# microsoft/Tokenizer

Measured on AMD Instinct MI355X. Metric: input MB/s encoded (cl100k_base), higher is better.
Workload: dtype u8

## Files before the change

### tokenizer_amd/csrc/tkz_kernels.hip

```cpp
#include "tkz_kernels.h"

#include <type_traits>

#include "tkz_bpe.h"
#include "tkz_classes.h"
#include "tkz_corpus.h"
#include "tkz_pretok.h"
#include "tkz_simt.h"

namespace tkz {

TKZ_KERNEL(256) void k_docmark(const int64_t* offs, int64_t n_items, int64_t total, uint64_t* bits, int32_t* counters) {
    const int64_t stride = simt::nblocks() * simt::nthreads();
    for (int64_t d = simt::bid() * simt::nthreads() + simt::tid(); d <= n_items; d += stride) {
        const int64_t pos = offs[d];
        bool ok = pos >= 0 && pos <= total;
        if (d == 0) ok = ok && pos == 0;
        if (d == n_items) ok = ok && pos == total;
        else ok = ok && pos <= offs[d + 1];
        if (!ok) { simt::atomic_or((unsigned*)&counters[0], (unsigned)kErrOffsets); continue; }
        const int64_t w = pos >> 6;
        if (d > 0) { const int64_t prev = offs[d - 1]; if (prev >= 0 && prev <= pos && (prev >> 6) == w) continue; }
        uint64_t m = 1ull << (pos & 63);
        int64_t cur = pos;
// ... 1311 lines not shown
    int* s_cls = LD.cls;
    uint16_t* s_ord = LD.ord;
    const int lane = simt::lane();
    int err = 0;
    LongProf PF;
    tkz_long_prof_begin(P, PF);
    const int64_t nchunks = (P.nsub + 63) / 64;
    for (int64_t u = c0; u < nchunks * PARTS; u += cstep) {
        const int64_t c = u % nchunks;
        const int part = (int)(u / nchunks);
        const int64_t t = c * 64 + lane;
        int my_nl = 0;
        if (t < P.nsub) {
            const uint32_t mc = P.mcount[t];
            my_nl = (int)(mc >> 16);
            if ((int)(mc & 0xFFFFu) + my_nl > P.mcap) my_nl = 0;
            if (part == 0 && (P.heavy_flag[t] & 2u)) { const int g = P.giant_cnt[t]; if (g > 1) simt::atomic_add(&P.tile_count[t], g - 1); }
        }
        int ntotal;
        (void)tkz_wave_scan_sum(my_nl, &ntotal);
        if (ntotal > DENSE) { if (lane / (64 / PARTS) != part) my_nl = 0; }
        else if (part != 0) continue;
        const int pre = tkz_wave_scan_sum(my_nl, &ntotal);
        if (!ntotal) continue;
        (void)simt::ballot(true);
        s_pre[lane] = pre;
        if (lane == 0) s_pre[64] = ntotal;
        (void)simt::ballot(true);
        auto entry_at = [&](int g, int* q, int* j) -> uint32_t {
            *q = tkz_find_list<64>(s_pre, g); *j = g - s_pre[*q];
            return tkz_load_nt(&P.mlist[(c * 64 + *q) * (int64_t)P.mcap + (P.mcap - 1 - *j)]);
        };
#ifdef TKZ_DEVPROF
        if (PF.on) { ++PF.units; PF.t0 = simt::clock(); }
#endif
        for (int seg0 = 0; seg0 < ntotal; seg0 += kLongSeg) {
            const int nseg = ntotal - seg0 < kLongSeg ? ntotal - seg0 : kLongSeg;
            if (lane < kLenClasses) s_cls[lane] = 0;
            (void)simt::ballot(true);
            uint32_t mycls = 0;
#pragma unroll
            for (int i = 0; i < kLongSeg / 64; ++i) {
                const int e = lane + 64 * i;
                if (e < nseg) {
                    int q, j;
                    const uint32_t ent = entry_at(seg0 + e, &q, &j);
                    const int cl = tkz_len_class((int)((ent >> kMrLenShift) & 1023u) + 1);
                    mycls |= (uint32_t)cl << (4 * i);
                    simt::atomic_add(&s_cls[cl], 1);
                }
            }
            (void)simt::ballot(true);
            {
                int tot;
                const int v = lane < kLenClasses ? s_cls[lane] : 0;
                const int x = tkz_wave_scan_sum(v, &tot);
                (void)simt::ballot(true);
                if (lane < kLenClasses) s_cls[lane] = x;
            }
            (void)simt::ballot(true);
#pragma unroll
            for (int i = 0; i < kLongSeg / 64; ++i) {
                const int e = lane + 64 * i;
                if (e < nseg) s_ord[simt::atomic_add(&s_cls[(mycls >> (4 * i)) & 15u], 1)] = (uint16_t)e;
            }
            (void)simt::ballot(true);
            TKZ_PF_MARK(0);
            for (int done = 0; done < nseg;) {
                const bool valid = done + lane < nseg;
                int q = 0, j = 0, len = 1, rel = 0;
                if (valid) {
                    const uint32_t ent = entry_at(seg0 + (int)s_ord[done + lane], &q, &j);
                    rel = (int)(ent & 1023u); len = (int)((ent >> kMrLenShift) & 1023u) + 1;
                }
                const int64_t sub = c * 64 + q;
                const int limit = tkz_long_batch<COMPACT>(T, P, LD, valid, sub, j, rel, len, lane_piece, err, PF, [](int) {});
                (void)simt::ballot(true);
                done += limit < nseg - done ? limit : nseg - done;
            }
        }
    }
    if (err) simt::atomic_or((unsigned*)&P.counters[0], (unsigned)err);
    tkz_long_prof_end(P, PF);
}
constexpr int kLongPartsLatency = 16;

constexpr int kLqRange = 256, kLqRangeLong = 16;
#ifndef TKZ_QARENA_DWORDS
#define TKZ_QARENA_DWORDS 2304
#endif
constexpr int kQArenaDwords = TKZ_QARENA_DWORDS;
static_assert(kQArenaDwords % 4 == 0 && kQArenaDwords >= (kLanePiece + 3) / 4 + 8 + 2 * kLanePiece + 16, "a piece of kLanePiece bytes fits the arena in every form");
#ifdef TKZ_HOSTEMU
constexpr int kLongQGrid = 8;
#else
constexpr int kLongQGrid = 8192;
#endif
template <class F>
TKZ_DEV void tkz_long_walk(const EncodeParams& P, int64_t c, int lane_piece, F f) {
    const int64_t t = c * 64 + simt::lane();
    int nl = 0;
    if (t < P.nsub) {
        const uint32_t mc = P.mcount[t];
        nl = (int)(mc >> 16);
        if ((int)(mc & 0xFFFFu) + nl > P.mcap) nl = 0;
    }
    const uint32_t* top = &P.mlist[t * (int64_t)P.mcap + (P.mcap - 1)];
    for (int j = 0; j < nl; j += 4) {
        uint32_t ent[4];
#pragma unroll
        for (int k = 0; k < 4; ++k) ent[k] = j + k < nl ? tkz_load_nt(top - (j + k)) : 0xFFFFFFFFu;
#pragma unroll
        for (int k = 0; k < 4; ++k) if (j + k < nl && !(ent[k] & kMrDone) && (int)((ent[k] >> kMrLenShift) & 1023u) + 1 <= lane_piece) f(t, j + k, ent[k]);
    }
}
TKZ_KERNEL(256) void k_long_count(EncodeParams P) {
    if (tkz_attempt_failed(P)) return;
    TKZ_SHARED int s_hist[4][kLenClasses];
    const int lane = simt::lane(), wave = simt::wave();
    const int64_t nchunks = (P.nsub + 63) / 64;
    for (int64_t c = simt::bid() * 4 + wave; c < nchunks; c += simt::nblocks() * 4) {
        if (lane < kLenClasses) s_hist[wave][lane] = 0;
        (void)simt::ballot(true);
        tkz_long_walk(P, c, P.lane_piece, [&](int64_t, int, uint32_t ent) { simt::atomic_add(&s_hist[wave][tkz_len_class((int)((ent >> kMrLenShift) & 1023u) + 1)], 1); });
        (void)simt::ballot(true);
        if (lane < kLenClasses) P.lq_cnt[(int64_t)lane * nchunks + c] = s_hist[wave][lane];
        (void)simt::ballot(true);
    }
}
TKZ_KERNEL(256) void k_long_scatter(EncodeParams P) {
    if (tkz_attempt_failed(P)) return;
    TKZ_SHARED int s_hist[4][kLenClasses];
    const int lane = simt::lane(), wave = simt::wave();
    const int64_t nchunks = (P.nsub + 63) / 64;
    for (int64_t c = simt::bid() * 4 + wave; c < nchunks; c += simt::nblocks() * 4) {
        if (lane < kLenClasses) s_hist[wave][lane] = 0;
        (void)simt::ballot(true);
        { const int64_t t = c * 64 + lane; if (t < P.nsub && (P.heavy_flag[t] & 2u)) { const int g = P.giant_cnt[t]; if (g > 1) simt::atomic_add(&P.tile_count[t], g - 1); } }
        tkz_long_walk(P, c, P.lane_piece, [&](int64_t t, int j, uint32_t ent) {
            const int cl = tkz_len_class((int)((ent >> kMrLenShift) & 1023u) + 1);
            const int64_t at = P.lq_base[(int64_t)cl * nchunks + c] + simt::atomic_add(&s_hist[wave][cl], 1);
            if (at < P.lq_cap) P.lq[at] = ((uint64_t)t << 30) | ((uint64_t)j << 20) | (uint64_t)(ent & 0xFFFFFu);
        });
        (void)simt::ballot(true);
    }
}
template <bool COMPACT>
TKZ_KERNEL_OCC(64, 4) void k_merge_long_q(TkzTables T, EncodeParams P) {
    if (tkz_attempt_failed(P)) return;
    TKZ_SHARED uint4 s_lds[(kQArenaDwords + 256) / 4];
    LongLds LD;
    LD.arena = reinterpret_cast<uint32_t*>(s_lds); LD.arena_dwords = kQArenaDwords; LD.brank = reinterpret_cast<int32_t*>(s_lds) + kQArenaDwords;
    LD.pre = nullptr; LD.cls = nullptr; LD.ord = nullptr;
    tkz_long_brank_init(T, LD.brank);
    const int lane = simt::lane();
    int err = 0;
    LongProf PF;
    tkz_long_prof_begin(P, PF);
    const int64_t total = *P.lq_total < P.lq_cap ? *P.lq_total : P.lq_cap;
    const int64_t nchunks = (P.nsub + 63) / 64;
    int64_t nfast = P.lq_base[(int64_t)tkz_len_class(kFastPiece + 1) * nchunks];
    if (nfast > total) nfast = total;
    int64_t rfast = kLqRange;
    while (rfast > 64 && (nfast + rfast - 1) / rfast < simt::nblocks()) rfast >>= 1;
    const int64_t nrf = (nfast + rfast - 1) / rfast, nrl = (total - nfast + kLqRangeLong - 1) / kLqRangeLong;
    auto range_of = [&](int64_t r, int64_t* lo, int64_t* hi) {
        if (r >= nrf) { *lo = nfast + (r - nrf) * kLqRangeLong; *hi = *lo + kLqRangeLong < total ? *lo + kLqRangeLong : total; }
        else { *lo = r * rfast; *hi = *lo + rfast < nfast ? *lo + rfast : nfast; }
    };
    auto entry_of = [&](int64_t pos, int64_t hi) -> uint64_t { return pos < hi ? P.lq[pos] : 0ull; };
    int64_t rg = nrf + nrl - 1 - simt::bid();
    int64_t lo = 0, hi = 0;
    if (rg >= 0) range_of(rg, &lo, &hi);
    uint64_t ent = rg >= 0 ? entry_of(lo + lane, hi) : 0ull;
    while (rg >= 0) {
#ifdef TKZ_DEVPROF
        if (PF.on) { ++PF.units; PF.t0 = simt::clock(); }
#endif
        int64_t nlo = 0, nhi = 0;
        const int64_t nrg = rg - simt::nblocks();
        if (nrg >= 0) range_of(nrg, &nlo, &nhi);
        for (int64_t at = lo; at < hi;) {
            const bool valid = at + lane < hi;
            const int64_t sub = valid ? (int64_t)(ent >> 30) : 0;
            const int j = valid ? (int)((ent >> 20) & 1023u) : 0, len = valid ? (int)((ent >> 10) & 1023u) + 1 : 1, rel = valid ? (int)(ent & 1023u) : 0;
            uint64_t ent_next = 0;
            TKZ_PF_MARK(0);
            const int limit = tkz_long_batch<COMPACT>(T, P, LD, valid, sub, j, rel, len, P.lane_piece, err, PF, [&](int n) {
                const int64_t nx = at + n;
                ent_next = nx < hi ? entry_of(nx + lane, hi) : (nrg >= 0 ? entry_of(nlo + lane, nhi) : 0ull);
            });
            at += limit;
            ent = ent_next;
        }
        rg = nrg; lo = nlo; hi = nhi;
    }
    if (err) simt::atomic_or((unsigned*)&P.counters[0], (unsigned)err);
    tkz_long_prof_end(P, PF);
}

constexpr int kCoopScratch = (4 * kTailSubs + 8) * 64 + 16 + 16;
constexpr int kCoopLdsBytes = 2 * 4 * kArenaPiece + 4 * (kArenaPiece / 32) + kCoopScratch;
#ifdef TKZ_HOSTEMU
constexpr int kCoopGrid = 4;
#else
constexpr int kCoopGrid = 2048;
#endif
constexpr int kCoopLdsQuads = (kCoopLdsBytes + 15) / 16;
TKZ_DEV void tkz_merge_coop_queue(const TkzTables& T, const EncodeParams& P, uint4* s_lds, unsigned long long bid, unsigned long long nblocks) {
    int32_t* ids = reinterpret_cast<int32_t*>(s_lds);
    int32_t* pr = ids + kArenaPiece;
    uint32_t* alive = reinterpret_cast<uint32_t*>(pr + kArenaPiece);
    uint8_t* scratch = reinterpret_cast<uint8_t*>(alive + kArenaPiece / 32);
    const int lane = simt::lane();
    int err = 0;
    const unsigned long long count = *P.coop_count < (unsigned long long)P.coop_cap ? *P.coop_count : (unsigned long long)P.coop_cap;
    bool first = true;
    for (;;) {
        unsigned long long tk = bid;
        if (!first) {
            if (lane == 0) tk = nblocks + simt::atomic_add64(P.coop_ticket, 1ull);
            tk = ((unsigned long long)simt::shflu((uint32_t)(tk >> 32), 0) << 32) | simt::shflu((uint32_t)tk, 0);
        }
        first = false;
        if (tk >= count) break;
        const uint64_t qe = P.coop_q[tk];
        const int64_t sub = (int64_t)(qe >> 10);
        const int jj = (int)(qe & 1023u);
        const uint32_t ee = P.mlist[sub * (int64_t)P.mcap + (P.mcap - 1 - jj)];
        if (ee & kMrDone) continue;
        const int rel = (int)(ee & 1023u), n = (int)((ee >> kMrLenShift) & 1023u) + 1;
        const int64_t abs = sub * kSub + rel;
        const uint8_t* gb = P.bytes + abs;
        for (int k = lane; k < n; k += 64) {
            const uint32_t b = gb[k];
            ids[k] = T.byte_rank[b];
            pr[k] = (k + 1 < n) ? T.bytepair_rank[(b << 8) | gb[k + 1]] : TKZ_RANK_NONE;
        }
        simt::sync();
        tkz_bpe_long_tail<true>(T, n, ids, pr, alive, scratch, nullptr);
        const int cnt = tkz_bpe_long_tail_emit<true>(n, ids, pr, alive, P.tmp + abs, &err);
        if (lane == 0) {
            P.mlist[sub * (int64_t)P.mcap + (P.mcap - 1 - jj)] = tkz_result_entry(false, cnt, rel);
            if (cnt > 1) simt::atomic_add(&P.tile_count[sub], cnt - 1);
        }
        simt::sync();
    }
    if (err) simt::atomic_or((unsigned*)&P.counters[0], (unsigned)err);
}
TKZ_KERNEL(64) void k_merge_coop(TkzTables T, EncodeParams P) {
    if (tkz_attempt_failed(P)) return;
    TKZ_SHARED uint4 s_lds[kCoopLdsQuads];
    tkz_merge_coop_queue(T, P, s_lds, (unsigned long long)simt::bid(), (unsigned long long)simt::nblocks());
}

constexpr int kMergeLatWaveQuads = kMsLdsQuads > kLongLdsQuads ? kMsLdsQuads : kLongLdsQuads;
template <bool COMPACT>
TKZ_KERNEL_OCC(kMsThreads, 3) void k_merge_latency(TkzTables T, EncodeParams P, int nb_short, int nb_long) {
    if (tkz_attempt_failed(P)) return;
    TKZ_SHARED uint4 s_wave[kMsThreads / 64][kMergeLatWaveQuads];
    TKZ_SHARED uint16_t s_brank16[256];
    const int b = (int)simt::bid();
    if (b < nb_short) {
        tkz_ms_brank_init(T, s_brank16);
        simt::sync();
        const int64_t grp = tkz_xcd_block(b, nb_short) * (kMsThreads / 64) + simt::wave();
        tkz_merge_short_group(T, P, grp, tkz_ms_lds(s_wave[simt::wave()], s_brank16));
    } else {
        const LongLds LD = tkz_long_lds(s_wave[simt::wave()]);
        tkz_long_brank_init(T, LD.brank);
        tkz_merge_long_chunks<COMPACT, kLongPartsLatency, -1>(T, P, (int64_t)(b - nb_short) * (kMsThreads / 64) + simt::wave(), (int64_t)nb_long * (kMsThreads / 64), LD, P.lane_piece);
    }
}

#ifndef TKZ_PLACE_OCC
#define TKZ_PLACE_OCC 7
#endif
constexpr int kPlacePer = 4;
constexpr int kPlaceBig = 8;
#ifndef TKZ_PLACE_FAST_BIG
#define TKZ_PLACE_FAST_BIG 64
#endif
constexpr int kPlaceFastBig = TKZ_PLACE_FAST_BIG;
constexpr int kStageMin = 64 * kPlaceBig + 16;
#ifndef TKZ_PLACE_STAGE
#define TKZ_PLACE_STAGE 784
#endif
constexpr int kStageBatch = TKZ_PLACE_STAGE;
static_assert(kStageBatch >= kStageMin && kStageBatch % 16 == 0, "whole quads, and room for one batch of the general path");
template <int SLOTS, int STAGE> constexpr int kPlaceLdsQuadsT = STAGE / 4 + SLOTS + SLOTS / 4 + 1 + SLOTS / 4;
constexpr int kPlaceLdsQuads = kPlaceLdsQuadsT<64, kStageMin>;
struct PlaceLds { int32_t* stage; uint4* quad; uint32_t* res; int32_t* pos; };
template <int SLOTS, int STAGE>
TKZ_DEV PlaceLds tkz_place_lds(uint4* wave_quads) {
    constexpr int kStage = STAGE;
    PlaceLds L;
    L.stage = reinterpret_cast<int32_t*>(wave_quads);
    L.quad = wave_quads + kStage / 4;
    L.res = reinterpret_cast<uint32_t*>(wave_quads + kStage / 4 + SLOTS);
    L.pos = reinterpret_cast<int32_t*>(wave_quads + kStage / 4 + SLOTS + SLOTS / 4 + 1);
    return L;
}
template <int SLOTS, bool PROMO, int STAGE>
TKZ_DEV void tkz_place_subtiles(const EncodeParams& P, const int64_t* tile_base, int32_t* out, int64_t out_cap, int64_t sub0, const PlaceLds& LD) {
    constexpr int kPlaceSlots = SLOTS, kPlaceRes = SLOTS / 2, kStage = STAGE;
    const int lane = simt::lane();
    if (sub0 >= P.nsub) return;
    int32_t* stage = LD.stage;
    uint32_t* s_res = LD.res;
    uint4* s_quad = LD.quad;
    int32_t* s_pos = LD.pos;
    struct Sc { int64_t pb, tb, ord0; int np; uint32_t mc, hf; int gc; };
    auto load_sc = [&](int64_t sub) -> Sc {
        Sc c;
        c.pb = P.pbase[sub]; c.tb = tile_base[sub]; c.ord0 = P.docord_base[sub]; c.np = P.pcount[sub]; c.mc = P.mcount[sub]; c.hf = P.heavy_flag[sub]; c.gc = P.giant_cnt[sub];
        return c;
    };
    Sc nxt = load_sc(sub0);
    auto load_recs = [&](int64_t pb_, int np_, int kk, uint32_t* r) {
        const int k0 = kk + 4 * lane;
        r[0] = r[1] = r[2] = r[3] = 0u;
        if (k0 < np_) {
            if (pb_ + k0 + 4 <= P.prank_cap) { const uint4 v = tkz_load16_nt(&P.prank[pb_ + k0]); r[0] = v.x; r[1] = v.y; r[2] = v.z; r[3] = v.w; }
            else for (int j = 0; j < 4; ++j) if (pb_ + k0 + j < P.prank_cap) r[j] = (uint32_t)P.prank[pb_ + k0 + j];
        }
    };
#pragma unroll 1
    for (int it = 0; it < kPlacePer && sub0 + it < P.nsub; ++it) {
    const int64_t sub = sub0 + it;
    const Sc cur = nxt;
    if (it + 1 < kPlacePer && sub + 1 < P.nsub) nxt = load_sc(sub + 1);
    const int64_t pb = cur.pb, tb = cur.tb, base = sub * kSub, ord0 = cur.ord0;
    const int np = cur.np;
    const uint32_t mc = cur.mc;
    const int ns = (int)(mc & 0xFFFFu), nl = (int)(mc >> 16);
    const uint32_t* const ml = P.mlist + sub * (int64_t)P.mcap;
    const uint4* const mqd = P.mquad + sub * (int64_t)P.mcap;
    const int32_t* const dense = P.dense + (sub / kGroup) * kDenseCap;
    const bool has_giant = (cur.hf & 2u) != 0;
    int gcnt = has_giant ? cur.gc : 0;
    if (gcnt < 0) gcnt = 0;
    const bool lists_ok = ns + nl <= P.mcap;
    static_assert(SLOTS == 64 || SLOTS == 128, "one or two kept entries per lane: slots lane and lane + 64");
    const int kl = ns + nl <= kPlaceSlots ? nl : (nl < kPlaceRes ? nl : kPlaceRes), ks = ns < kPlaceSlots - kl ? ns : kPlaceSlots - kl;
    const bool two = SLOTS == 128 && ks + kl > 64;
    const int top = two ? kPlaceSlots - 1 : 63;
    bool fast_ok;
    {
        uint32_t a[2] = {0u, 0u};
        uint4 qd[2];
        bool big = false;
#pragma unroll
        for (int h = 0; h < 2; ++h) {
            qd[h].x = qd[h].y = qd[h].z = qd[h].w = 0;
            if (h == 1 && !two) break;
            const int slot = lane + 64 * h;
            const bool shortside = slot < ks;
            const int e = shortside ? slot : top - slot;
            const bool want = lists_ok && (shortside || e < kl);
            const int64_t at = shortside ? e : P.mcap - 1 - e;
            if (want) { a[h] = tkz_load_nt(&ml[at]); qd[h] = tkz_load16_nt(&mqd[at]); }
            big = big || (want && tkz_result_cnt(a[h]) > kPlaceFastBig);
        }
        (void)simt::ballot(true);
        s_res[lane] = a[0]; s_quad[lane] = qd[0]; s_pos[lane] = -1;
        if constexpr (SLOTS == 128) { s_res[lane + 64] = a[1]; s_quad[lane + 64] = qd[1]; s_pos[lane + 64] = -1; }
        if (lane == 0) s_res[kPlaceSlots] = tkz_result_inline(1);
        fast_ok = lists_ok && !has_giant && ns + nl <= kPlaceSlots && !simt::ballot(big);
    }
    (void)simt::ballot(true);
    auto answer = [&](uint32_t rec) -> uint32_t {
        if (rec & kPrGiant) return tkz_result_entry(false, 1, (int)(rec & 1023u));
        const int idx = (int)(rec & 1023u);
        const bool lg = (rec & kPrLong) != 0;
        if (!lists_ok) return tkz_result_inline(1);
        return (lg ? idx < kl : idx < ks) ? s_res[lg ? top - idx : idx] : ml[lg ? P.mcap - 1 - idx : idx];
    };
    auto inline_quad = [&](uint32_t rec) -> uint4 {
        const int idx = (int)(rec & 1023u);
        const bool lg = (rec & kPrLong) != 0;
        if (!lists_ok) { uint4 z; z.x = z.y = z.z = z.w = 0; return z; }
        return (lg ? idx < kl : idx < ks) ? s_quad[lg ? top - idx : idx] : tkz_load16(&mqd[lg ? P.mcap - 1 - idx : idx]);
    };
    auto token_src = [&](uint32_t res) -> const int32_t* { return (res & kMrDense) ? dense + tkz_result_off(res) : P.tmp + base + tkz_result_off(res); };
    const uintptr_t out_addr = reinterpret_cast<uintptr_t>(out);
    auto quad_base = [&](int tok) -> int { return tok - (int)(((out_addr >> 2) + (uintptr_t)(tb + tok)) & 3u); };
    int running = 0, marks = 0, flushed = 0, sbase = quad_base(0);
    auto flush = [&](int upto) {
        (void)simt::ballot(true);
        const int lo = flushed - sbase, hi = upto - sbase;
        for (int q4 = lane; 4 * q4 < hi; q4 += 64) {
            const int i0 = 4 * q4;
            if (i0 + 4 <= lo) continue;
            const uint4 v = reinterpret_cast<const uint4*>(stage)[q4];
            int32_t* dst = out + tb + sbase + i0;
            if (i0 >= lo && i0 + 4 <= hi && tb + sbase + i0 + 4 <= out_cap) tkz_store16_nt(dst, v);
            else {
                const int32_t w[4] = {(int32_t)v.x, (int32_t)v.y, (int32_t)v.z, (int32_t)v.w};
#pragma unroll
                for (int i = 0; i < 4; ++i) if (i0 + i >= lo && i0 + i < hi && tb + sbase + i0 + i < out_cap) dst[i] = w[i];
            }
        }
        (void)simt::ballot(true);
        flushed = upto; sbase = quad_base(upto);
    };
    auto place_fast = [&](int kk) -> bool {
        const int k0 = kk + 4 * lane;
        uint32_t r[4];
        load_recs(pb, np, kk, r);
        int c[4], idx[4];
        bool ok[4], ms[4], pm[4];
        uint4 pq0;
        int pj = -1, pdst = 0, pcnt = 0;
        int t = 0, mk = 0;
        if constexpr (PROMO) {
#pragma unroll
            for (int j = 3; j >= 0; --j) { pm[j] = k0 + j < np && pb + k0 + j < P.prank_cap && !(r[j] & kPrMiss) && (r[j] & kPromoFlag); if (pm[j]) pj = j; }
            pq0 = tkz_load16(&P.promo[pj >= 0 ? (r[pj >= 0 ? pj : 0] & kPromoIdxMask) : 0u]);
        }
#pragma unroll
        for (int j = 0; j < 4; ++j) {
            ok[j] = k0 + j < np && pb + k0 + j < P.prank_cap;
            ms[j] = ok[j] && (r[j] & kPrMiss);
            idx[j] = ((r[j] & kPrLong) ? top - (int)(r[j] & 1023u) : (int)(r[j] & 1023u)) & (kPlaceSlots - 1);
            const uint32_t a = s_res[ms[j] ? idx[j] : kPlaceSlots];
            c[j] = ok[j] ? tkz_result_cnt(a) : 0;
            if constexpr (PROMO) { if (pm[j]) c[j] = (int)((r[j] >> kPromoCntShift) & 3u) + 1; }
            t += c[j];
            mk += (ok[j] && (r[j] & kPrMark)) ? 1 : 0;
        }
        int both;
        const int pre = tkz_wave_scan_sum(t | (mk << 20), &both);
        const int tot = both & 0xFFFFF, mtot = both >> 20;
        if (running + tot - sbase > kStage) {
            if (flushed < running) flush(running);
            if (running + tot - sbase > kStage) return false;
        }
        int pos = running + (pre & 0xFFFFF), mi = marks + (pre >> 20);
#pragma unroll
        for (int j = 0; j < 4; ++j) {
            if (ok[j] && (r[j] & kPrMark)) P.doc_tok[ord0 + mi++] = pos;
            if (ms[j]) s_pos[idx[j]] = pos;
            else if (PROMO && pm[j]) {
                if (j == pj) { pdst = pos - sbase; pcnt = c[j]; }
                else {
                    const uint4 q = tkz_load16(&P.promo[r[j] & kPromoIdxMask]);
                    int32_t* dst = stage + (pos - sbase);
                    dst[0] = (int32_t)q.x;
                    if (c[j] > 1) dst[1] = (int32_t)q.y;
                    if (c[j] > 2) dst[2] = (int32_t)q.z;
                    if (c[j] > 3) dst[3] = (int32_t)q.w;
                }
            }
            else if (ok[j]) stage[pos - sbase] = (int32_t)(r[j] & kPrRankMask);
            pos += c[j];
        }
        (void)simt::ballot(true);
#pragma unroll
        for (int h = 0; h < 2; ++h) {
            if (h == 1 && !two) break;
            const int slot = lane + 64 * h;
            const int p = s_pos[slot];
            if (p >= 0) {
                const uint32_t ans = s_res[slot];
                const int cnt = tkz_result_cnt(ans);
                int32_t* dst = stage + (p - sbase);
                if (ans & kMrInline) {
                    const uint4 q = s_quad[slot];
                    dst[0] = (int32_t)q.x;
                    if (cnt > 1) dst[1] = (int32_t)q.y;
                    if (cnt > 2) dst[2] = (int32_t)q.z;
                    if (cnt > 3) dst[3] = (int32_t)q.w;
                } else {
                    const int32_t* src = token_src(ans);
                    for (int i = 0; i < cnt; ++i) dst[i] = src[i];
                }
                s_pos[slot] = -1;
            }
        }
        if constexpr (PROMO) {
            if (pcnt) {
                int32_t* dst = stage + pdst;
                dst[0] = (int32_t)pq0.x;
                if (pcnt > 1) dst[1] = (int32_t)pq0.y;
                if (pcnt > 2) dst[2] = (int32_t)pq0.z;
                if (pcnt > 3) dst[3] = (int32_t)pq0.w;
            }
        }
        running += tot; marks += mtot;
        return true;
    };
#pragma unroll 1
    for (int kk = 0; kk < np; kk += 256) {
      if (fast_ok && place_fast(kk)) continue;
#pragma unroll 1
      for (int j = 0; j < 4; ++j) {
        const int k0 = kk + 64 * j;
        if (k0 >= np) break;
        const int k = k0 + lane;
        const bool valid = k < np && pb + k < P.prank_cap;
        const uint32_t rec = valid ? (uint32_t)tkz_load_nt(&P.prank[pb + k]) : 0u;
        const uint32_t res = (rec & kPrMiss) ? answer(rec) : 0u;
        const bool miss = (rec & kPrMiss) != 0;
        const bool promoted = PROMO && valid && !miss && (rec & kPromoFlag);
        uint4 pquad; pquad.x = pquad.y = pquad.z = pquad.w = 0;
        if constexpr (PROMO) { if (promoted) pquad = tkz_load16(&P.promo[rec & kPromoIdxMask]); }
        const int cnt = !valid ? 0 : !miss ? (promoted ? (int)((rec >> kPromoCntShift) & 3u) + 1 : 1) : (rec & kPrGiant) ? gcnt : tkz_result_cnt(res);
        int tot;
        const int pos = running + tkz_wave_scan_sum(cnt, &tot);
        const uint64_t mm = simt::ballot(valid && (rec & kPrMark));
        if (valid && (rec & kPrMark)) P.doc_tok[ord0 + marks + tkz_popc64(mm & tkz_lowmask(lane))] = pos;
        const uint64_t big = simt::ballot(valid && miss && cnt > kPlaceBig);
        if (!big) {
            if (running + tot - sbase > kStage) flush(running);
            if (valid) {
                int32_t* dst = stage + (pos - sbase);
                if (promoted) {
                    dst[0] = (int32_t)pquad.x;
                    if (cnt > 1) dst[1] = (int32_t)pquad.y;
                    if (cnt > 2) dst[2] = (int32_t)pquad.z;
                    if (cnt > 3) dst[3] = (int32_t)pquad.w;
                }
                else if (!miss) dst[0] = (int32_t)(rec & kPrRankMask);
                else if (res & kMrInline) {
                    const uint4 q = inline_quad(rec);
                    dst[0] = (int32_t)q.x;
                    if (cnt > 1) dst[1] = (int32_t)q.y;
                    if (cnt > 2) dst[2] = (int32_t)q.z;
                    if (cnt > 3) dst[3] = (int32_t)q.w;
                } else {
                    const int32_t* src = token_src(res);
                    for (int i = 0; i < cnt; ++i) dst[i] = src[i];
                }
            }
        } else {
            flush(running);
            const int32_t* src = (miss && !(res & kMrInline)) ? token_src(res) : nullptr;
            if (valid) {
                int32_t* dst = out + tb + pos;
                if (promoted) {
                    const int32_t w[4] = {(int32_t)pquad.x, (int32_t)pquad.y, (int32_t)pquad.z, (int32_t)pquad.w};
#pragma unroll
                    for (int i = 0; i < 4; ++i) if (i < cnt && tb + pos + i < out_cap) dst[i] = w[i];
                }
                else if (!miss) { if (tb + pos < out_cap) tkz_store_nt(&dst[0], (int32_t)(rec & kPrRankMask)); }
                else if (res & kMrInline) {
                    const uint4 q = inline_quad(rec);
                    const int32_t w[4] = {(int32_t)q.x, (int32_t)q.y, (int32_t)q.z, (int32_t)q.w};
#pragma unroll
                    for (int i = 0; i < 4; ++i) if (i < cnt && tb + pos + i < out_cap) dst[i] = w[i];
                } else if (cnt <= kPlaceBig) {
                    for (int i = 0; i < cnt; ++i) if (tb + pos + i < out_cap) dst[i] = src[i];
                }
            }
            for (uint64_t bg = big; bg; bg &= bg - 1) {
                const int src_lane = tkz_ctz64(bg);
                const int c = simt::shfl(cnt, src_lane), p0 = simt::shfl(pos, src_lane);
                const uint32_t lo32 = simt::shflu((uint32_t)(reinterpret_cast<uintptr_t>(src)), src_lane), hi32 = simt::shflu((uint32_t)(reinterpret_cast<uintptr_t>(src) >> 32), src_lane);
                const int32_t* bsrc = reinterpret_cast<const int32_t*>(((uintptr_t)hi32 << 32) | lo32);
                int32_t* dst = out + tb + p0;
                for (int i = lane; i < c; i += 64) if (tb + p0 + i < out_cap) dst[i] = bsrc[i];
            }
            flushed = running + tot; sbase = quad_base(flushed);
        }
        running += tot;
        marks += tkz_popc64(mm);
      }
    }
    if (flushed < running) flush(running);
    }
}
template <int SLOTS, bool PROMO>
TKZ_KERNEL_OCC(256, TKZ_PLACE_OCC) void k_place(EncodeParams P, const int64_t* tile_base, int32_t* out, int64_t out_cap) {
    if (tkz_attempt_failed(P)) return;
    TKZ_SHARED uint4 s_wave[kThreads / 64][kPlaceLdsQuadsT<SLOTS, kStageBatch>];
    const int64_t sub0 = (tkz_xcd_block(simt::bid(), simt::nblocks()) * (kThreads / 64) + simt::wave()) * kPlacePer;
    tkz_place_subtiles<SLOTS, PROMO, kStageBatch>(P, tile_base, out, out_cap, sub0, tkz_place_lds<SLOTS, kStageBatch>(s_wave[simt::wave()]));
}

constexpr int kCountSlots = 128, kCountLaneMax = (1 << 20) / 64 - 1;
#ifndef TKZ_TOKCOUNT_OCC
#define TKZ_TOKCOUNT_OCC 8
#endif
TKZ_KERNEL_OCC(256, TKZ_TOKCOUNT_OCC) void k_tokcount(EncodeParams P, const int32_t* dcount) {
    if (tkz_attempt_failed(P)) return;
    TKZ_SHARED int32_t s_wave[kThreads / 64][kCountSlots + 4];
    const int lane = simt::lane();
    int32_t* const s_cnt = s_wave[simt::wave()];
    const int64_t sub0 = (tkz_xcd_block(simt::bid(), simt::nblocks()) * (kThreads / 64) + simt::wave()) * kPlacePer;
    if (sub0 >= P.nsub) return;
    const bool promo = P.promo != nullptr;
    struct Sc { int64_t pb, ord0; int np, dc; uint32_t mc, hf; int gc; };
    auto load_sc = [&](int64_t sub) -> Sc {
        Sc c;
        c.dc = dcount[sub]; c.pb = P.pbase[sub]; c.ord0 = P.docord_base[sub]; c.np = P.pcount[sub]; c.mc = P.mcount[sub]; c.hf = P.heavy_flag[sub]; c.gc = P.giant_cnt[sub];
        return c;
    };
    Sc nxt = load_sc(sub0);
#pragma unroll 1
    for (int it = 0; it < kPlacePer && sub0 + it < P.nsub; ++it) {
        const int64_t sub = sub0 + it;
        const Sc cur = nxt;
        if (it + 1 < kPlacePer && sub + 1 < P.nsub) nxt = load_sc(sub + 1);
        const int dc = cur.dc;
        if (dc <= 0) continue;
        const int64_t pb = cur.pb, ord0 = cur.ord0;
        const int np = cur.np;
        const int ns = (int)(cur.mc & 0xFFFFu), nl = (int)(cur.mc >> 16);
        const uint32_t* const ml = P.mlist + sub * (int64_t)P.mcap;
        const bool has_giant = (cur.hf & 2u) != 0;
        int gcnt = has_giant ? cur.gc : 0;
        if (gcnt < 0) gcnt = 0;
        const bool lists_ok = ns + nl <= P.mcap;
        const int kl = ns + nl <= kCountSlots ? nl : (nl < kCountSlots / 2 ? nl : kCountSlots / 2), ks = ns < kCountSlots - kl ? ns : kCountSlots - kl;
        const bool two = ks + kl > 64;
        const int top = two ? kCountSlots - 1 : 63;
        {
            int a[2] = {1, 1};
#pragma unroll
            for (int h = 0; h < 2; ++h) {
                if (h == 1 && !two) break;
                const int slot = lane + 64 * h;
                const bool shortside = slot < ks;
                const int e = shortside ? slot : top - slot;
                if (lists_ok && (shortside || e < kl)) a[h] = tkz_result_cnt(tkz_load_nt(&ml[shortside ? e : P.mcap - 1 - e]));
            }
            (void)simt::ballot(true);
            s_cnt[lane] = a[0]; s_cnt[lane + 64] = a[1];
            if (lane == 0) s_cnt[kCountSlots] = 1;
        }
        (void)simt::ballot(true);
        const bool all_kept = lists_ok && !has_giant && ns + nl <= kCountSlots;
        auto miss_count = [&](uint32_t rec) -> int {
            if (rec & kPrGiant) return gcnt;
            if (!lists_ok) return 1;
            const int idx = (int)(rec & 1023u);
            const bool lg = (rec & kPrLong) != 0;
            if (lg ? idx < kl : idx < ks) return s_cnt[lg ? top - idx : idx];
            return idx < P.mcap ? tkz_result_cnt(ml[lg ? P.mcap - 1 - idx : idx]) : 1;
        };
        int running = 0, marks = 0;
#pragma unroll 1
        for (int kk = 0; kk < np && marks < dc; kk += 256) {
            const int k0 = kk + 4 * lane;
            uint32_t r[4] = {0u, 0u, 0u, 0u};
            if (k0 < np) {
                if (pb + k0 + 4 <= P.prank_cap) { const uint4 v = tkz_load16_nt(&P.prank[pb + k0]); r[0] = v.x; r[1] = v.y; r[2] = v.z; r[3] = v.w; }
                else for (int j = 0; j < 4; ++j) if (pb + k0 + j < P.prank_cap) r[j] = (uint32_t)P.prank[pb + k0 + j];
            }
            int c[4];
            bool mkd[4];
            int t = 0, mk = 0;
#pragma unroll
            for (int j = 0; j < 4; ++j) {
                const bool ok = k0 + j < np && pb + k0 + j < P.prank_cap;
                const bool ms = ok && (r[j] & kPrMiss);
                if (all_kept) {
                    const int idx = ((r[j] & kPrLong) ? top - (int)(r[j] & 1023u) : (int)(r[j] & 1023u)) & (kCountSlots - 1);
                    c[j] = ok ? s_cnt[ms ? idx : kCountSlots] : 0;
                } else c[j] = !ok ? 0 : ms ? miss_count(r[j]) : 1;
                if (promo && ok && !ms && (r[j] & kPromoFlag)) c[j] = (int)((r[j] >> kPromoCntShift) & 3u) + 1;
                mkd[j] = ok && (r[j] & kPrMark);
                t += c[j];
                mk += mkd[j] ? 1 : 0;
            }
            if (!simt::ballot(t > kCountLaneMax)) {
                int both;
                const int pre = tkz_wave_scan_sum(t | (mk << 20), &both);
                int pos = running + (pre & 0xFFFFF), mi = marks + (pre >> 20);
#pragma unroll
                for (int j = 0; j < 4; ++j) {
                    if (mkd[j] && mi < dc) P.doc_tok[ord0 + mi] = pos;
                    mi += mkd[j] ? 1 : 0;
                    pos += c[j];
                }
                running += both & 0xFFFFF; marks += both >> 20;
                continue;
            }
#pragma unroll 1
            for (int j = 0; j < 4 && marks < dc; ++j) {
                const int q0 = kk + 64 * j;
                if (q0 >= np) break;
                const int k = q0 + lane;
                const bool valid = k < np && pb + k < P.prank_cap;
                const uint32_t rec = valid ? (uint32_t)tkz_load_nt(&P.prank[pb + k]) : 0u;
                const bool miss = (rec & kPrMiss) != 0;
                int cnt = !valid ? 0 : miss ? miss_count(rec) : 1;
                if (promo && valid && !miss && (rec & kPromoFlag)) cnt = (int)((rec >> kPromoCntShift) & 3u) + 1;
                int tot;
                const int pos = running + tkz_wave_scan_sum(cnt, &tot);
                const bool marked = valid && (rec & kPrMark);
                const uint64_t mm = simt::ballot(marked);
                const int mi = marks + tkz_popc64(mm & tkz_lowmask(lane));
                if (marked && mi < dc) P.doc_tok[ord0 + mi] = pos;
                running += tot;
                marks += tkz_popc64(mm);
            }
        }
    }
}

TKZ_DEV void tkz_giant_find_one(int64_t t, const uint64_t* startbits, int64_t nwords, int64_t total, int64_t* gq, unsigned long long* gcount, int64_t gcap) {
    int64_t p = -1;
    for (int k = kSub / 64 - 1; k >= 0 && p < 0; --k) {
        const int64_t w = t * (kSub / 64) + k;
        const uint64_t m = w < nwords ? startbits[w] : 0;
        if (m) p = (w << 6) + tkz_msb64(m);
    }
    if (p < 0 || p >= total) return;
    int64_t next = total;
    for (int64_t v = (t + 1) * (kSub / 64); v < nwords; ++v) {
        const uint64_t x = startbits[v];
        if (x) { next = (v << 6) + tkz_ctz64(x); break; }
    }
    if (next - p > kArenaPiece) {
        const unsigned long long q = simt::atomic_add64(gcount, 1ull);
        if ((int64_t)q < gcap) { gq[2 * q] = p; gq[2 * q + 1] = next - p; }
    }
}
constexpr int kGiantSort = 8192;
TKZ_KERNEL(1024) void k_giant_order(EncodeParams P) {
    if (tkz_attempt_failed(P)) return;
    TKZ_SHARED int32_t s_len[kGiantSort];
    const int64_t n = (int64_t)*P.giant_count < P.giant_cap ? (int64_t)*P.giant_count : P.giant_cap;
    int64_t* order = P.giant_q + 2 * P.giant_cap;
    if (n > kGiantSort) { for (int64_t i = simt::tid(); i < n; i += simt::nthreads()) order[i] = i; return; }
    for (int i = simt::tid(); i < (int)n; i += simt::nthreads()) { const int64_t l = P.giant_q[2 * i + 1]; s_len[i] = l > 0x7FFFFFFF ? 0x7FFFFFFF : (int32_t)l; }
    simt::sync();
    for (int i = simt::tid(); i < (int)n; i += simt::nthreads()) {
        const int32_t li = s_len[i];
        int rank = 0;
        for (int j = 0; j < (int)n; ++j) { const int32_t lj = s_len[j]; rank += (lj > li || (lj == li && j < i)) ? 1 : 0; }
        order[rank] = i;
    }
}

TKZ_KERNEL(1024) void k_giant_merge(TkzTables T, EncodeParams P) {
    if (tkz_attempt_failed(P)) return;
    TKZ_SHARED alignas(16) int32_t s_state[kBpeLongLdsBytes / 4];
    TKZ_SHARED int64_t s_off;
    TKZ_SHARED int32_t s_whole;
    TKZ_SHARED unsigned long long s_ticket;
    const int64_t n = (int64_t)*P.giant_count < P.giant_cap ? (int64_t)*P.giant_count : P.giant_cap;
    const int64_t* order = P.giant_q + 2 * P.giant_cap;
    int err = 0;
    for (;;) {
        if (simt::tid() == 0) s_ticket = simt::atomic_add64(P.giant_ticket, 1ull);
        simt::sync();
        const int64_t t = (int64_t)s_ticket;
        simt::sync();
        if (t >= n) break;
        const int64_t q = order[t];
        const int64_t p = P.giant_q[2 * q], len64 = P.giant_q[2 * q + 1];
        int cnt = 0;
        if (len64 > kMaxPiece) err |= kErrTooLong;
        else {
            const int len = (int)len64;
            const uint8_t* gb = P.bytes + p;
            auto at = [&](int i) -> uint32_t { return gb[i]; };
            int32_t* dst = P.tmp + p;
            if (simt::tid() == 0) {
                s_whole = tkz_lookup_long(T, at, (uint32_t)len);
                const unsigned long long need = 6ull * (unsigned long long)len;
                const unsigned long long o = simt::atomic_add64(P.pool_head, need);
                s_off = (o + need <= (unsigned long long)P.pool_cap) ? (int64_t)o : -1;
            }
            simt::sync();
            const int32_t whole = s_whole;
            const int64_t off = s_off;
            simt::sync();
            if (whole != TKZ_RANK_NONE) { if (simt::tid() == 0) dst[0] = whole; cnt = 1; }
            else if (off < 0) { err |= kErrPool; cnt = -1; }
            else {
                int32_t* arr = P.pool + off;
                cnt = tkz_bpe_long(T, at, len, arr, arr + len, arr + 2 * (int64_t)len, arr + 3 * (int64_t)len, arr + 4 * (int64_t)len, arr + 5 * (int64_t)len, dst, &err, s_state, TKZ_DEV_FLAG(P, 16) ? P.devprof : nullptr);
            }
        }
        if (simt::tid() == 0) P.giant_cnt[p / kSub] = cnt;
        simt::sync();
    }
    if (err) simt::atomic_or((unsigned*)&P.counters[0], (unsigned)err);
}

TKZ_KERNEL(256) void k_doccount2(const uint64_t* bits_a, const uint64_t* bits_b, int64_t nwords, int64_t total, int64_t nsub, int32_t* cnt_a, int32_t* cnt_b) {
    static_assert(kSub / 64 == 16, "k_doccount2 sums 16 lanes per sub-tile");
    const int lane = simt::lane();
    const int64_t stride = simt::nblocks() * simt::nthreads(), nw = nsub * (kSub / 64);
    for (int64_t w0 = simt::bid() * simt::nthreads() + (simt::tid() & ~63); w0 < nw; w0 += stride) {
        const int64_t w = w0 + lane;
        uint64_t ma = (w < nw && w < nwords) ? bits_a[w] : 0ull, mb = (w < nw && w < nwords) ? bits_b[w] : 0ull;
        const int64_t lim = total - (w << 6);
        if (lim <= 0) { ma = 0; mb = 0; } else if (lim < 64) { ma &= tkz_lowmask((int)lim); mb &= tkz_lowmask((int)lim); }
        int c = tkz_popc64(ma) | (tkz_popc64(mb) << 16);
        c += simt::shfl_xor(c, 1); c += simt::shfl_xor(c, 2); c += simt::shfl_xor(c, 4); c += simt::shfl_xor(c, 8);
        if ((lane & 15) == 0 && w < nw) { cnt_a[w >> 4] = c & 0xFFFF; cnt_b[w >> 4] = c >> 16; }
    }
}

constexpr int kScanSmallMax = 8192;
TKZ_KERNEL(1024) void k_scan_small(const int32_t* cnt_a, int64_t* base_a, int64_t* grand_a, int round_a,
                                   const int32_t* cnt_b, int64_t* base_b, int64_t* grand_b, int round_b, int n) {
    const int tid = simt::tid(), nth = simt::nthreads();
    const int per = (n + nth - 1) / nth, lo = tid * per, hi = lo + per < n ? lo + per : n;
    for (int arr = 0; arr < 2; ++arr) {
        const int32_t* cnt = arr ? cnt_b : cnt_a;
        int64_t* base = arr ? base_b : base_a;
        int64_t* grand = arr ? grand_b : grand_a;
        const int round = arr ? round_b : round_a;
        if (!cnt) continue;
        int sum = 0;
        for (int i = lo; i < hi; ++i) sum += (cnt[i] + round) & ~round;
        int tot;
        int run = tkz_block_scan(sum, &tot);
        for (int i = lo; i < hi; ++i) { base[i] = run; run += (cnt[i] + round) & ~round; }
        if (tid == 0 && grand) *grand = tot;
        simt::sync();
    }
}
TKZ_KERNEL(256) void k_scan_partials(const int32_t* cnt, int64_t n, int64_t* bsum, int round) {
    TKZ_SHARED int64_t s_w[4];
    const int64_t i0 = simt::bid() * kScanBlock;
    int64_t v = 0;
    for (int j = simt::tid(); j < kScanBlock; j += kThreads) if (i0 + j < n) v += (cnt[i0 + j] + round) & ~round;
    for (int d = 32; d >= 1; d >>= 1) {
        const uint32_t lo = simt::shflu((uint32_t)v, simt::lane() ^ d), hi = simt::shflu((uint32_t)((uint64_t)v >> 32), simt::lane() ^ d);
        v += (int64_t)(((uint64_t)hi << 32) | lo);
    }
    if (simt::lane() == 0) s_w[simt::wave()] = v;
    simt::sync();
    if (simt::tid() == 0) bsum[simt::bid()] = s_w[0] + s_w[1] + s_w[2] + s_w[3];
}
TKZ_KERNEL(256) void k_scan_top(int64_t* bsum, int64_t nblk, int64_t* grand) {
    TKZ_SHARED int64_t s_w[kThreads / 64];
    const int lane = simt::lane(), wave = simt::wave();
    int64_t carry = 0;
    for (int64_t i0 = 0; i0 < nblk; i0 += kThreads) {
        const int64_t i = i0 + simt::tid();
        const int64_t v = i < nblk ? bsum[i] : 0;
        int64_t x = v;
        for (int d = 1; d < 64; d <<= 1) {
            const uint32_t lo = simt::shflu((uint32_t)x, lane - d < 0 ? lane : lane - d);
            const uint32_t hi = simt::shflu((uint32_t)((uint64_t)x >> 32), lane - d < 0 ? lane : lane - d);
            if (lane >= d) x += (int64_t)(((uint64_t)hi << 32) | lo);
        }
        if (lane == 63) s_w[wave] = x;
        simt::sync();
        int64_t woff = 0, tot = 0;
        for (int w = 0; w < kThreads / 64; ++w) { const int64_t t = s_w[w]; if (w < wave) woff += t; tot += t; }
        simt::sync();
        if (i < nblk) bsum[i] = carry + woff + x - v;
        carry += tot;
    }
    if (simt::tid() == 0) *grand = carry;
}
TKZ_KERNEL(256) void k_scan_final(const int32_t* cnt, int64_t n, const int64_t* boff, int64_t* base, int round) {
    const int64_t i0 = simt::bid() * kScanBlock;
    constexpr int per = kScanBlock / kThreads;
    int local[per]; int sum = 0;
    for (int j = 0; j < per; ++j) { const int64_t i = i0 + (int64_t)simt::tid() * per + j; local[j] = i < n ? (cnt[i] + round) & ~round : 0; sum += local[j]; }
    int tot;
    int pre = tkz_block_scan(sum, &tot);
    int64_t run = boff[simt::bid()] + pre;
    for (int j = 0; j < per; ++j) { const int64_t i = i0 + (int64_t)simt::tid() * per + j; if (i < n) base[i] = run; run += local[j]; }
}

TKZ_KERNEL(256) void k_docoffs(const int64_t* offs, int64_t n_docs, int64_t total, const int64_t* tile_base, const uint64_t* docbits,
                               const int64_t* docord_base, const int32_t* doc_tok, const int64_t* grand, int64_t* out_offs,
                               int64_t c3_docs, int64_t* c3a, int64_t* c3b, int64_t* c3c) {
    const int64_t stride = simt::nblocks() * simt::nthreads();
    if (simt::bid() == 0 && simt::tid() == 0) {
        const int64_t g = *grand;
        if (c3a) { c3a[0] = c3_docs; c3a[1] = total; c3a[2] = g; }
        if (c3b) { c3b[0] = c3_docs; c3b[1] = total; c3b[2] = g; }
        if (c3c) { c3c[0] = c3_docs; c3c[1] = total; c3c[2] = g; }
    }
    for (int64_t d = simt::bid() * simt::nthreads() + simt::tid(); d <= n_docs; d += stride) {
// ... 1429 lines not shown
```

Measured before the change: 269,600.

## Hoist per-subtile list and record loads in place kernel, scalarize bases

Restructures the placement kernel so the per-subtile scalar header is made wave-uniform through first-lane broadcasts. The kept-answer list loads and the first record batch are now issued before the next subtile's header prefetch. Bounds checks on prank, out and doc_tok are rewritten as 32-bit offsets from uniform base pointers with clamped room values, and the header arrays are passed as restrict pointers. The intent is to overlap global-load latency and cut 64-bit address arithmetic and VGPR use. It also lowers the occupancy bound for the 128-slot variant, trading waves per SIMD for more registers.

```diff
diff --git a/tokenizer_amd/csrc/tkz_kernels.hip b/tokenizer_amd/csrc/tkz_kernels.hip
--- a/tokenizer_amd/csrc/tkz_kernels.hip
+++ b/tokenizer_amd/csrc/tkz_kernels.hip
@@ -1637,7 +1637,9 @@
     return L;
 }
 template <int SLOTS, bool PROMO, int STAGE>
-TKZ_DEV void tkz_place_subtiles(const EncodeParams& P, const int64_t* tile_base, int32_t* out, int64_t out_cap, int64_t sub0, const PlaceLds& LD) {
+TKZ_DEV void tkz_place_subtiles_sc(const EncodeParams& P, int32_t* out, int64_t out_cap, int64_t sub0, const PlaceLds& LD,
+                                   const int64_t* __restrict__ pbase, const int64_t* __restrict__ tile_base, const int64_t* __restrict__ docord_base, const int32_t* __restrict__ pcount,
+                                   const uint32_t* __restrict__ mcount, const uint8_t* __restrict__ heavy_flag, const int32_t* __restrict__ giant_cnt) {
     constexpr int kPlaceSlots = SLOTS, kPlaceRes = SLOTS / 2, kStage = STAGE;
     const int lane = simt::lane();
     if (sub0 >= P.nsub) return;
@@ -1648,22 +1650,55 @@
     struct Sc { int64_t pb, tb, ord0; int np; uint32_t mc, hf; int gc; };
     auto load_sc = [&](int64_t sub) -> Sc {
         Sc c;
-        c.pb = P.pbase[sub]; c.tb = tile_base[sub]; c.ord0 = P.docord_base[sub]; c.np = P.pcount[sub]; c.mc = P.mcount[sub]; c.hf = P.heavy_flag[sub]; c.gc = P.giant_cnt[sub];
+        c.pb = pbase[sub]; c.tb = tile_base[sub]; c.ord0 = docord_base[sub]; c.np = pcount[sub]; c.mc = mcount[sub]; c.hf = heavy_flag[sub]; c.gc = giant_cnt[sub];
         return c;
     };
-    Sc nxt = load_sc(sub0);
     auto load_recs = [&](int64_t pb_, int np_, int kk, uint32_t* r) {
         const int k0 = kk + 4 * lane;
+        const int32_t* const recs = P.prank + pb_;
+        const int64_t room64 = P.prank_cap - pb_;
+        const int room = room64 < 0 ? 0 : room64 > (1 << 20) ? (1 << 20) : (int)room64;
         r[0] = r[1] = r[2] = r[3] = 0u;
         if (k0 < np_) {
-            if (pb_ + k0 + 4 <= P.prank_cap) { const uint4 v = tkz_load16_nt(&P.prank[pb_ + k0]); r[0] = v.x; r[1] = v.y; r[2] = v.z; r[3] = v.w; }
-            else for (int j = 0; j < 4; ++j) if (pb_ + k0 + j < P.prank_cap) r[j] = (uint32_t)P.prank[pb_ + k0 + j];
+            if (k0 + 4 <= room) { const uint4 v = tkz_load16_nt(&recs[(uint32_t)k0]); r[0] = v.x; r[1] = v.y; r[2] = v.z; r[3] = v.w; }
+            else for (int j = 0; j < 4; ++j) if (k0 + j < room) r[j] = (uint32_t)recs[(uint32_t)(k0 + j)];
         }
     };
+    static_assert(SLOTS == 64 || SLOTS == 128, "one or two kept entries per lane: slots lane and lane + 64");
+    struct Kept { int ks, kl, top; bool two, lists_ok; };
+    auto kept_of = [&](uint32_t mc_) -> Kept {
+        const int ns_ = (int)(mc_ & 0xFFFFu), nl_ = (int)(mc_ >> 16);
+        Kept k;
+        k.lists_ok = ns_ + nl_ <= P.mcap;
+        k.kl = ns_ + nl_ <= kPlaceSlots ? nl_ : (nl_ < kPlaceRes ? nl_ : kPlaceRes);
+        k.ks = ns_ < kPlaceSlots - k.kl ? ns_ : kPlaceSlots - k.kl;
+        k.two = SLOTS == 128 && k.ks + k.kl > 64;
+        k.top = k.two ? kPlaceSlots - 1 : 63;
+        return k;
+    };
+    auto load_ans = [&](int64_t sub_, const Kept& k, int h, uint32_t& a, uint4& qd) {
+        a = 0u; qd.x = qd.y = qd.z = qd.w = 0;
+        const int slot = lane + 64 * h;
+        const bool shortside = slot < k.ks;
+        const int e = shortside ? slot : k.top - slot;
+        const bool want = k.lists_ok && (shortside || e < k.kl);
+        const uint32_t at = (uint32_t)((shortside ? e : P.mcap - 1 - e) & (kMissCapMax - 1));
+        const uint32_t* const ml_ = P.mlist + sub_ * (int64_t)P.mcap;
+        const uint4* const mqd_ = P.mquad + sub_ * (int64_t)P.mcap;
+        if (want) { a = tkz_load_nt(&ml_[at]); qd = tkz_load16_nt(&mqd_[at]); }
+    };
+    Sc nxt = load_sc(sub0);
 #pragma unroll 1
     for (int it = 0; it < kPlacePer && sub0 + it < P.nsub; ++it) {
     const int64_t sub = sub0 + it;
-    const Sc cur = nxt;
+    Sc cur;
+    cur.pb = (int64_t)simt::uniform64((uint64_t)nxt.pb); cur.tb = (int64_t)simt::uniform64((uint64_t)nxt.tb); cur.ord0 = (int64_t)simt::uniform64((uint64_t)nxt.ord0);
+    cur.np = simt::first_lane(nxt.np); cur.mc = (uint32_t)simt::first_lane((int)nxt.mc); cur.hf = (uint32_t)simt::first_lane((int)nxt.hf); cur.gc = simt::first_lane(nxt.gc);
+    const Kept kp = kept_of(cur.mc);
+    uint32_t a[2] = {0u, 0u}, r_cur[4];
+    uint4 qd[2];
+    load_ans(sub, kp, 0, a[0], qd[0]);
+    load_recs(cur.pb, cur.np, 0, r_cur);
     if (it + 1 < kPlacePer && sub + 1 < P.nsub) nxt = load_sc(sub + 1);
     const int64_t pb = cur.pb, tb = cur.tb, base = sub * kSub, ord0 = cur.ord0;
     const int np = cur.np;
@@ -1675,28 +1710,14 @@
     const bool has_giant = (cur.hf & 2u) != 0;
     int gcnt = has_giant ? cur.gc : 0;
     if (gcnt < 0) gcnt = 0;
-    const bool lists_ok = ns + nl <= P.mcap;
-    static_assert(SLOTS == 64 || SLOTS == 128, "one or two kept entries per lane: slots lane and lane + 64");
-    const int kl = ns + nl <= kPlaceSlots ? nl : (nl < kPlaceRes ? nl : kPlaceRes), ks = ns < kPlaceSlots - kl ? ns : kPlaceSlots - kl;
-    const bool two = SLOTS == 128 && ks + kl > 64;
-    const int top = two ? kPlaceSlots - 1 : 63;
+    const bool lists_ok = kp.lists_ok;
+    const int kl = kp.kl, ks = kp.ks, top = kp.top;
+    const bool two = kp.two;
     bool fast_ok;
     {
-        uint32_t a[2] = {0u, 0u};
-        uint4 qd[2];
-        bool big = false;
-#pragma unroll
-        for (int h = 0; h < 2; ++h) {
-            qd[h].x = qd[h].y = qd[h].z = qd[h].w = 0;
-            if (h == 1 && !two) break;
-            const int slot = lane + 64 * h;
-            const bool shortside = slot < ks;
-            const int e = shortside ? slot : top - slot;
-            const bool want = lists_ok && (shortside || e < kl);
-            const int64_t at = shortside ? e : P.mcap - 1 - e;
-            if (want) { a[h] = tkz_load_nt(&ml[at]); qd[h] = tkz_load16_nt(&mqd[at]); }
-            big = big || (want && tkz_result_cnt(a[h]) > kPlaceFastBig);
-        }
+        qd[1].x = qd[1].y = qd[1].z = qd[1].w = 0;
+        if (two) load_ans(sub, kp, 1, a[1], qd[1]);
+        const bool big = tkz_result_cnt(a[0]) > kPlaceFastBig || tkz_result_cnt(a[1]) > kPlaceFastBig;
         (void)simt::ballot(true);
         s_res[lane] = a[0]; s_quad[lane] = qd[0]; s_pos[lane] = -1;
         if constexpr (SLOTS == 128) { s_res[lane + 64] = a[1]; s_quad[lane + 64] = qd[1]; s_pos[lane + 64] = -1; }
@@ -1724,25 +1745,32 @@
     auto flush = [&](int upto) {
         (void)simt::ballot(true);
         const int lo = flushed - sbase, hi = upto - sbase;
+        int32_t* const obase = reinterpret_cast<int32_t*>(simt::uniform64(reinterpret_cast<uintptr_t>(out + tb + sbase)));
+        const int64_t oroom64 = out_cap - tb - sbase;
+        const int oroom = oroom64 < 0 ? 0 : oroom64 > (1 << 20) ? (1 << 20) : (int)oroom64;
         for (int q4 = lane; 4 * q4 < hi; q4 += 64) {
             const int i0 = 4 * q4;
             if (i0 + 4 <= lo) continue;
             const uint4 v = reinterpret_cast<const uint4*>(stage)[q4];
-            int32_t* dst = out + tb + sbase + i0;
-            if (i0 >= lo && i0 + 4 <= hi && tb + sbase + i0 + 4 <= out_cap) tkz_store16_nt(dst, v);
+            int32_t* dst = obase + (uint32_t)i0;
+            if (i0 >= lo && i0 + 4 <= hi && i0 + 4 <= oroom) tkz_store16_nt(dst, v);
             else {
                 const int32_t w[4] = {(int32_t)v.x, (int32_t)v.y, (int32_t)v.z, (int32_t)v.w};
 #pragma unroll
-                for (int i = 0; i < 4; ++i) if (i0 + i >= lo && i0 + i < hi && tb + sbase + i0 + i < out_cap) dst[i] = w[i];
+                for (int i = 0; i < 4; ++i) if (i0 + i >= lo && i0 + i < hi && i0 + i < oroom) dst[i] = w[i];
             }
         }
         (void)simt::ballot(true);
         flushed = upto; sbase = quad_base(upto);
     };
+    const int64_t room64 = P.prank_cap - pb;
+    const int nrec = room64 < np ? (room64 < 0 ? 0 : (int)room64) : np;
+    int32_t* const doc_tok = P.doc_tok + ord0;
+    int32_t* const otile = reinterpret_cast<int32_t*>(simt::uniform64(reinterpret_cast<uintptr_t>(out + tb)));
     auto place_fast = [&](int kk) -> bool {
         const int k0 = kk + 4 * lane;
-        uint32_t r[4];
-        load_recs(pb, np, kk, r);
+        uint32_t r[4] = {r_cur[0], r_cur[1], r_cur[2], r_cur[3]};
+        if (kk) load_recs(pb, np, kk, r);
         int c[4], idx[4];
         bool ok[4], ms[4], pm[4];
         uint4 pq0;
@@ -1750,12 +1778,12 @@
         int t = 0, mk = 0;
         if constexpr (PROMO) {
 #pragma unroll
-            for (int j = 3; j >= 0; --j) { pm[j] = k0 + j < np && pb + k0 + j < P.prank_cap && !(r[j] & kPrMiss) && (r[j] & kPromoFlag); if (pm[j]) pj = j; }
+            for (int j = 3; j >= 0; --j) { pm[j] = k0 + j < nrec && !(r[j] & kPrMiss) && (r[j] & kPromoFlag); if (pm[j]) pj = j; }
             pq0 = tkz_load16(&P.promo[pj >= 0 ? (r[pj >= 0 ? pj : 0] & kPromoIdxMask) : 0u]);
         }
 #pragma unroll
         for (int j = 0; j < 4; ++j) {
-            ok[j] = k0 + j < np && pb + k0 + j < P.prank_cap;
+            ok[j] = k0 + j < nrec;
             ms[j] = ok[j] && (r[j] & kPrMiss);
             idx[j] = ((r[j] & kPrLong) ? top - (int)(r[j] & 1023u) : (int)(r[j] & 1023u)) & (kPlaceSlots - 1);
             const uint32_t a = s_res[ms[j] ? idx[j] : kPlaceSlots];
@@ -1774,7 +1802,7 @@
         int pos = running + (pre & 0xFFFFF), mi = marks + (pre >> 20);
 #pragma unroll
         for (int j = 0; j < 4; ++j) {
-            if (ok[j] && (r[j] & kPrMark)) P.doc_tok[ord0 + mi++] = pos;
+            if (ok[j] && (r[j] & kPrMark)) doc_tok[(uint32_t)mi++] = pos;
             if (ms[j]) s_pos[idx[j]] = pos;
             else if (PROMO && pm[j]) {
                 if (j == pj) { pdst = pos - sbase; pcnt = c[j]; }
@@ -1833,8 +1861,8 @@
         const int k0 = kk + 64 * j;
         if (k0 >= np) break;
         const int k = k0 + lane;
-        const bool valid = k < np && pb + k < P.prank_cap;
-        const uint32_t rec = valid ? (uint32_t)tkz_load_nt(&P.prank[pb + k]) : 0u;
+        const bool valid = k < nrec;
+        const uint32_t rec = valid ? (uint32_t)tkz_load_nt(&(P.prank + pb)[(uint32_t)k]) : 0u;
         const uint32_t res = (rec & kPrMiss) ? answer(rec) : 0u;
         const bool miss = (rec & kPrMiss) != 0;
         const bool promoted = PROMO && valid && !miss && (rec & kPromoFlag);
@@ -1844,7 +1872,7 @@
         int tot;
         const int pos = running + tkz_wave_scan_sum(cnt, &tot);
         const uint64_t mm = simt::ballot(valid && (rec & kPrMark));
-        if (valid && (rec & kPrMark)) P.doc_tok[ord0 + marks + tkz_popc64(mm & tkz_lowmask(lane))] = pos;
+        if (valid && (rec & kPrMark)) doc_tok[(uint32_t)(marks + tkz_popc64(mm & tkz_lowmask(lane)))] = pos;
         const uint64_t big = simt::ballot(valid && miss && cnt > kPlaceBig);
         if (!big) {
             if (running + tot - sbase > kStage) flush(running);
@@ -1872,7 +1900,7 @@
             flush(running);
             const int32_t* src = (miss && !(res & kMrInline)) ? token_src(res) : nullptr;
             if (valid) {
-                int32_t* dst = out + tb + pos;
+                int32_t* dst = otile + (uint32_t)pos;
                 if (promoted) {
                     const int32_t w[4] = {(int32_t)pquad.x, (int32_t)pquad.y, (int32_t)pquad.z, (int32_t)pquad.w};
 #pragma unroll
@@ -1893,7 +1921,7 @@
                 const int c = simt::shfl(cnt, src_lane), p0 = simt::shfl(pos, src_lane);
                 const uint32_t lo32 = simt::shflu((uint32_t)(reinterpret_cast<uintptr_t>(src)), src_lane), hi32 = simt::shflu((uint32_t)(reinterpret_cast<uintptr_t>(src) >> 32), src_lane);
                 const int32_t* bsrc = reinterpret_cast<const int32_t*>(((uintptr_t)hi32 << 32) | lo32);
-                int32_t* dst = out + tb + p0;
+                int32_t* dst = otile + (uint32_t)p0;
                 for (int i = lane; i < c; i += 64) if (tb + p0 + i < out_cap) dst[i] = bsrc[i];
             }
             flushed = running + tot; sbase = quad_base(flushed);
@@ -1905,8 +1933,12 @@
     if (flushed < running) flush(running);
     }
 }
+template <int SLOTS, bool PROMO, int STAGE>
+TKZ_DEV void tkz_place_subtiles(const EncodeParams& P, const int64_t* tile_base, int32_t* out, int64_t out_cap, int64_t sub0, const PlaceLds& LD) {
+    tkz_place_subtiles_sc<SLOTS, PROMO, STAGE>(P, out, out_cap, sub0, LD, P.pbase, tile_base, P.docord_base, P.pcount, P.mcount, P.heavy_flag, P.giant_cnt);
+}
 template <int SLOTS, bool PROMO>
-TKZ_KERNEL_OCC(256, TKZ_PLACE_OCC) void k_place(EncodeParams P, const int64_t* tile_base, int32_t* out, int64_t out_cap) {
+TKZ_KERNEL_OCC(256, SLOTS == 128 && TKZ_PLACE_OCC > 6 ? 6 : TKZ_PLACE_OCC) void k_place(EncodeParams P, const int64_t* tile_base, int32_t* out, int64_t out_cap) {
     if (tkz_attempt_failed(P)) return;
     TKZ_SHARED uint4 s_wave[kThreads / 64][kPlaceLdsQuadsT<SLOTS, kStageBatch>];
     const int64_t sub0 = (tkz_xcd_block(simt::bid(), simt::nblocks()) * (kThreads / 64) + simt::wave()) * kPlacePer;
```

After: 274,800, median of 6. +1.9%, better.
